# python-hydro/pyro2

Hardware: AMD Instinct MI355X
Metric: cell-updates/s (higher is better)
Workload: dtype f64; 1 GPU; compressible sedov 16384x16384 (inputs.sedov physics: HLLC, limiter 2, flattening, cvisc 0.1, cfl 0.8, outflow), one GPU, single domain (no decomposition, no halo exchange); parallelism=slab1, halo=none, fast_math=1, kernel_set=-1, dt_policy=device, state=steps 5-362 from t = 0

## Files before the change

### include/pyrohip.h

```cpp
#ifndef PYROHIP_H
#define PYROHIP_H

#include <stddef.h>

#ifdef __cplusplus
extern "C" {
#endif

typedef struct pyrohip_ctx pyrohip_ctx;
typedef struct pyrohip_state pyrohip_state;
typedef struct pyrohip_mg pyrohip_mg;

enum {
    PYROHIP_BC_OUTFLOW = 0,
    PYROHIP_BC_REFLECT_EVEN = 1,
    PYROHIP_BC_REFLECT_ODD = 2,
    PYROHIP_BC_PERIODIC = 3,
    PYROHIP_BC_HALO = 4,
    PYROHIP_BC_HSE = 5,
    PYROHIP_BC_AMBIENT = 6,
    PYROHIP_BC_RAMP = 7,
    PYROHIP_BC_CONST = 8
};

// ... 99 lines not shown
                         const double *dts, int nsteps);
int pyrohip_advrk_stage_dump(pyrohip_state *s, int var, const pyrohip_advrk_params *p, int method,
                             double dt, int stage, double *host);

typedef struct {
    double dx, dy;
    double gamma;
    int limiter;
    int use_flattening;
    double z0, z1, delta;
    double cvisc;
    double grav;
    double small_dens;
    int avisc_xhi_interior, avisc_yhi_interior;
    int fast_math;
    int kernel_set;
    int riemann, solid_xl, solid_yl;
    int do_sponge;
    double sponge_rho_begin, sponge_rho_full, sponge_timescale;
    double heat_rate;
    int march_rows;
    int fuse_fill;
    int step_launches;
} pyrohip_comp_params;

int pyrohip_comp_dt(pyrohip_state *s, const pyrohip_comp_params *p, double cfl,
                    double *dt_out);
int pyrohip_comp_step(pyrohip_state *s, const pyrohip_comp_params *p,
                      double dt);
int pyrohip_comp_wave_geometry(int nx, int ny, int ng, int num_cus, int march_rows, int *out6);
typedef struct {
    double tmax, init_tstep_factor, max_dt_change, fix_dt;
    double t, dt_old;
    long long n;
} pyrohip_dt_policy;
int pyrohip_comp_evolve(pyrohip_state *s, const pyrohip_comp_params *p, double cfl,
                        pyrohip_dt_policy *policy, int max_steps, int *steps_done,
                        double *dts_out);
int pyrohip_comp_stage_dump(pyrohip_state *s, int stage_id, double *out);

int pyrohip_mg_create(pyrohip_ctx *ctx, int nx, double xmin, double xmax,
                      double ymin, double ymax, const int *bc, double alpha,
                      double beta, int nsmooth, int nsmooth_bottom,
                      pyrohip_mg **out);
int pyrohip_mg_destroy(pyrohip_mg *m);
int pyrohip_mg_set_helmholtz(pyrohip_mg *m, double alpha, double beta);
int pyrohip_mg_nlevels(pyrohip_mg *m, int *nlevels);
int pyrohip_mg_set_smoother(pyrohip_mg *m, int kind);
typedef struct {
    int kmax, kmax_small, nsmall;
    int march_min, march_waves;
    double march_side;
    int march_minrows;
// ... 147 lines not shown
```

### pyro2_amd/_lib.py

```python
import ctypes as C
import os
import threading

import numpy as np

HERE = os.path.dirname(os.path.abspath(__file__))
DEFAULT_LIB = os.path.join(HERE, "lib", "libpyrohip.so")

BC_OUTFLOW, BC_REFLECT_EVEN, BC_REFLECT_ODD, BC_PERIODIC, BC_HALO, BC_HSE, BC_AMBIENT, BC_RAMP, \
    BC_CONST = range(9)
BC_CODE = {"outflow": BC_OUTFLOW, "neumann": BC_OUTFLOW,
           "reflect-even": BC_REFLECT_EVEN, "reflect-odd": BC_REFLECT_ODD,
           "dirichlet": BC_REFLECT_ODD, "periodic": BC_PERIODIC,
           "halo": BC_HALO, "hse": BC_HSE, "ambient": BC_AMBIENT, "ramp": BC_RAMP,
           "moving_lid": BC_CONST}

class GeomArrays(C.Structure):
    NAMES = ("Lx", "Ly", "Ax", "Ay", "V", "dlogAx", "dlogAy", "x2d", "sint", "sinb", "sinc")
    _fields_ = [(n, C.POINTER(C.c_double)) for n in NAMES] + \
               [("xmin", C.c_double), ("ymin", C.c_double),
                ("rowf", C.POINTER(C.c_double)), ("colf", C.POINTER(C.c_double))]


ERR_STATE = 10002
# ... 27 lines not shown
class MGTuning(C.Structure):
    _fields_ = [("kmax", C.c_int), ("kmax_small", C.c_int), ("nsmall", C.c_int),
                ("march_min", C.c_int), ("march_waves", C.c_int), ("march_side", C.c_double),
                ("march_minrows", C.c_int), ("fuse_res_restrict", C.c_int),
                ("lazy_residual", C.c_int), ("allow_pow2", C.c_int), ("small_tiles", C.c_int),
                ("band_maxn", C.c_int), ("band_genedge", C.c_int), ("coarse_band64", C.c_int),
                ("speculate", C.c_int), ("trace", C.c_int), ("spec_debug", C.c_int),
                ("march_tail", C.c_int), ("coarse_wave", C.c_int)]


class CompParams(C.Structure):
    _fields_ = [("dx", C.c_double), ("dy", C.c_double), ("gamma", C.c_double),
                ("limiter", C.c_int), ("use_flattening", C.c_int),
                ("z0", C.c_double), ("z1", C.c_double), ("delta", C.c_double),
                ("cvisc", C.c_double), ("grav", C.c_double),
                ("small_dens", C.c_double),
                ("avisc_xhi_interior", C.c_int),
                ("avisc_yhi_interior", C.c_int),
                ("fast_math", C.c_int), ("kernel_set", C.c_int),
                ("riemann", C.c_int), ("solid_xl", C.c_int), ("solid_yl", C.c_int),
                ("do_sponge", C.c_int), ("sponge_rho_begin", C.c_double),
                ("sponge_rho_full", C.c_double), ("sponge_timescale", C.c_double),
                ("heat_rate", C.c_double), ("march_rows", C.c_int), ("fuse_fill", C.c_int),
                ("step_launches", C.c_int)]


class DtPolicyC(C.Structure):
    _fields_ = [("tmax", C.c_double), ("init_tstep_factor", C.c_double),
                ("max_dt_change", C.c_double), ("fix_dt", C.c_double),
                ("t", C.c_double), ("dt_old", C.c_double), ("n", C.c_longlong)]


_DP = C.POINTER(C.c_double)
_IP = C.POINTER(C.c_int)
_VP = C.c_void_p

_PROTOS = {
    "pyrohip_init": [C.c_int, C.POINTER(_VP)],
    "pyrohip_shutdown": [_VP],
    "pyrohip_sync": [_VP],
    "pyrohip_device_info": [_VP, C.c_char_p, C.c_int, C.POINTER(C.c_size_t),
                            C.POINTER(C.c_size_t), _IP],
    "pyrohip_prof_enable": [_VP, C.c_int],
    "pyrohip_prof_report": [_VP, C.c_char_p, C.c_int],
    "pyrohip_timer_start": [_VP],
    "pyrohip_timer_stop": [_VP, _DP],
    "pyrohip_state_create": [_VP, C.c_int, C.c_int, C.c_int, C.c_int, _IP,
# ... 50 lines not shown
                                C.c_double, C.c_double, C.c_double, C.c_int],
    "pyrohip_inc_stage_dump": [_VP, C.c_int, _DP],
    "pyrohip_lm_set_base": [_VP, _DP, _DP, _DP, _DP],
    "pyrohip_lm_dt": [_VP, C.c_double, C.c_double, C.c_double, C.c_double, _DP],
    "pyrohip_lm_mg_coeffs": [_VP, _VP],
    "pyrohip_lm_mac_rhs": [_VP, _VP, C.c_double, C.c_double, C.c_double, C.c_int, C.c_double, _DP],
    "pyrohip_lm_advect": [_VP, _VP, C.c_double, C.c_double, C.c_double, C.c_int, C.c_int,
                          C.c_double, C.c_double],
    "pyrohip_lm_proj_rhs": [_VP, _VP, C.c_double, C.c_double, C.c_double, C.c_int, C.c_int, _DP],
    "pyrohip_lm_proj_update": [_VP, _VP, C.c_double, C.c_double, C.c_double, C.c_int],
    "pyrohip_lm_stage_dump": [_VP, C.c_int, _DP],
    "pyrohip_fill_bc": [_VP, C.c_int],
    "pyrohip_state_set_user_bc": [_VP, C.c_double, C.c_double, C.c_double, _DP],
    "pyrohip_state_set_heating": [_VP, _DP],
    "pyrohip_state_set_source": [_VP, C.c_int, _VP],
    "pyrohip_comp_source_correct": [_VP, C.POINTER(CompParams), C.c_double],
    "pyrohip_state_set_ramp_bc": [_VP, _DP, C.c_double, _DP, _DP, _DP, _DP],
    "pyrohip_state_minmax": [_VP, C.c_int, C.c_int, _DP, _DP],
    "pyrohip_adv_step": [_VP, C.c_int, C.c_double, C.c_double, C.c_double,
                         C.c_double, C.c_double, C.c_int],
    "pyrohip_adv_step_fill": [_VP, C.c_int, C.c_double, C.c_double, C.c_double,
                              C.c_double, C.c_double, C.c_int, C.c_int],
    "pyrohip_adv_step_p": [_VP, C.c_int, C.POINTER(AdvParams), C.c_double],
    "pyrohip_comp_wave_geometry": [C.c_int, C.c_int, C.c_int, C.c_int, C.c_int, C.POINTER(C.c_int)],
    "pyrohip_adv_evolve": [_VP, C.c_int, C.POINTER(AdvParams), C.POINTER(C.c_double), C.c_int],
    "pyrohip_advnu_step": [_VP, C.c_int, C.c_int, C.c_int, C.POINTER(AdvNuParams), C.c_double],
    "pyrohip_advnu_evolve": [_VP, C.c_int, C.c_int, C.c_int, C.POINTER(AdvNuParams),
                             C.POINTER(C.c_double), C.c_int],
    "pyrohip_advnu_dt": [_VP, C.c_int, C.c_int, C.c_double, C.c_double, C.c_double, _DP],
    "pyrohip_advnu_stage_dump": [_VP, C.c_int, C.c_int, C.c_int, C.POINTER(AdvNuParams), C.c_double, _DP],
    "pyrohip_advrk_rhs": [_VP, C.c_int, C.POINTER(AdvRkParams), _VP, C.c_int],
    "pyrohip_advrk_step": [_VP, C.c_int, C.POINTER(AdvRkParams), C.c_int, C.c_double],
    "pyrohip_advrk_evolve": [_VP, C.c_int, C.POINTER(AdvRkParams), C.c_int, C.POINTER(C.c_double), C.c_int],
    "pyrohip_advrk_stage_dump": [_VP, C.c_int, C.POINTER(AdvRkParams), C.c_int, C.c_double, C.c_int, _DP],
    "pyrohip_comp_dt": [_VP, C.POINTER(CompParams), C.c_double, _DP],
    "pyrohip_comp_evolve": [_VP, C.POINTER(CompParams), C.c_double, C.POINTER(DtPolicyC), C.c_int,
                            _IP, _DP],
    "pyrohip_comp_step": [_VP, C.POINTER(CompParams), C.c_double],
    "pyrohip_comp_stage_dump": [_VP, C.c_int, _DP],
    "pyrohip_mg_create": [_VP, C.c_int, C.c_double, C.c_double, C.c_double,
                          C.c_double, _IP, C.c_double, C.c_double, C.c_int,
                          C.c_int, C.POINTER(_VP)],
    "pyrohip_mg_destroy": [_VP],
    "pyrohip_mg_nlevels": [_VP, _IP],
    "pyrohip_mg_set_smoother": [_VP, C.c_int],
    "pyrohip_mg_set": [_VP, C.c_int, C.c_int, _DP],
# ... 110 lines not shown
```

### pyro2_amd/csrc/common.h

```cpp
#pragma once
#include <hip/hip_runtime.h>

#include <cstdio>
#include <cstring>
#include <string>
#include <vector>

#include "../../include/pyrohip.h"

namespace pyro {

void set_error(const std::string &msg);

#define PYRO_CHECK_HIP(expr)                                                  \
    do {                                                                      \
        hipError_t _e = (expr);                                               \
        if (_e != hipSuccess) {                                               \
            ::pyro::set_error(std::string(#expr) + ": " +                     \
                              hipGetErrorString(_e));                         \
            return (int)_e;                                                   \
        }                                                                     \
    } while (0)

#define PYRO_REQUIRE(cond, msg)                                               \
// ... 186 lines not shown
    double *heat_base = nullptr, *heat = nullptr;
    const double *ext_old = nullptr, *ext_new = nullptr;
    int ext_pending = 0;
    bool ramp_bc = false, ramp_set = false;
    double *d_x = nullptr;
    double r_cxoff = 0.0, r_post[4] = {0, 0, 0, 0}, r_pre[4] = {0, 0, 0, 0};
    double r_sfd[8] = {0}, r_sfu[8] = {0};
    double *work = nullptr;
    size_t work_planes = 0;
    int *d_flag = nullptr;
    pyro::StepScalars *d_scal = nullptr;
    double *d_dts = nullptr;
    int dts_cap = 0;
    double *pend_part = nullptr;
    int pend_n = 0;
    double *d_cval = nullptr;
    pyro::SphGeom *sph = nullptr;
    int nb_lo = -1, nb_hi = -1;
    bool nb_set = false, halo_pending = false;
    bool frame_prefilled = false;
    pyro::StepPolicy *pol_next = nullptr;
    int pol_m = 0;
    unsigned long long *d_polmem = nullptr;
    double next_cfl_min = -1.0;
    bool cfl_is_global = false;
    int cfl_kind = 0;
    double cfl_par[3] = {0.0, 0.0, 0.0};
    bool ghost_by_rules = false;
    bool stages_valid = false;
};

inline int prio_board_acquire(pyrohip_ctx *c, int **board, int *tag)
{
    const size_t bytes = (size_t)2 * 65536 * sizeof(int);
    if (c->prio_board.bytes < bytes) {
        PYRO_TRY(c->prio_board.ensure(bytes));
        PYRO_CHECK_HIP(hipMemsetAsync(c->prio_board.p, 0, bytes, c->stream));
    }
    c->launch_seq = (c->launch_seq % 32767u) + 1u;
    *board = (int *)c->prio_board.p;
    *tag = (int)c->launch_seq;
    return 0;
}
inline int wave_fill_extra(int ncb, int nsb, int nx, int slots)
{
    const int nreg = ncb * nsb;
// ... 10 lines not shown
```

### pyro2_amd/csrc/comp_api.hip

```cpp
#include "common.h"
#include "stencil.h"

namespace pyro {
namespace exact {
int comp_dt(pyrohip_state *, const pyrohip_comp_params *, double, double *);
int comp_step_staged(pyrohip_state *, const pyrohip_comp_params *, double);
int comp_step_fused(pyrohip_state *, const pyrohip_comp_params *, double);
int comp_step_wave(pyrohip_state *, const pyrohip_comp_params *, double);
int comp_step_fused_ex(pyrohip_state *, const pyrohip_comp_params *, double, const StepScalars *,
                       const double **);
int comp_step_wave_ex(pyrohip_state *, const pyrohip_comp_params *, double, const StepScalars *,
                      const double **);
int comp_cfl_min_device(pyrohip_state *, const pyrohip_comp_params *, const double **);
int comp_step_sph(pyrohip_state *, const pyrohip_comp_params *, double);
int comp_step_wave_sph(pyrohip_state *, const pyrohip_comp_params *, double);
int comp_step_wave_sph_ex(pyrohip_state *, const pyrohip_comp_params *, double, const StepScalars *,
                          const double **);
int comp_step_fused_sph(pyrohip_state *, const pyrohip_comp_params *, double);
int comp_step_fused_sph_ex(pyrohip_state *, const pyrohip_comp_params *, double, const StepScalars *,
                           const double **);
int comp_cfl_min_device_sph(pyrohip_state *, const pyrohip_comp_params *, const double **);
int comp_dt_sph(pyrohip_state *, const pyrohip_comp_params *, double, double *);
int comp_stage_dump(pyrohip_state *, int, double *);
int comp_sponge(pyrohip_state *, const pyrohip_comp_params *, double);
// ... 817 lines not shown
    PYRO_REQUIRE(dst && src && k && slots_q && cq, "NULL argument");
    PYRO_REQUIRE(dst->nvar == src->nvar && dst->g.plane == src->g.plane && dst->g.plane == k->g.plane &&
                     dst->g.nx == k->g.nx && dst->g.ny == k->g.ny,
                 "geometries differ");
    PYRO_REQUIRE(dst->ctx == src->ctx && dst->ctx == k->ctx, "states live on different contexts");
    const int nslots = k->nvar / dst->nvar;
    PYRO_REQUIRE(slot_new >= 0 && slot_new < nslots && slot_old >= 0 && slot_old < nslots,
                 "slot outside the k state");
    for (int q = 0; q < 3; q++) PYRO_REQUIRE(slots_q[q] >= 0 && slots_q[q] < nslots, "slot outside the k state");
    PYRO_TRY(exact::comp_sdc_update(dst, src, k, slot_new, slot_old, slots_q, cq, dt));
    dst->next_cfl_min = -1.0;
    dst->ghost_by_rules = false;
    return 0;
}

int pyrohip_comp_stage_dump(pyrohip_state *s, int stage_id, double *out)
{
    PYRO_REQUIRE(s && out, "NULL argument");
    return exact::comp_stage_dump(s, stage_id, out);
}

}

extern "C" int pyrohip_comp_wave_geometry(int nx, int ny, int ng, int num_cus, int march_rows, int *out6)
{
    PYRO_REQUIRE(out6 && nx > 0 && ny > 0 && ng >= 0, "bad argument");
    return pyro::exact::comp_wave_geometry(nx, ny, ng, num_cus, march_rows, out6);
}
```

### pyro2_amd/csrc/comp_fused.hip

```cpp
#include "common.h"
#include "hydro.h"
#include "reduce.h"

#ifndef PYRO_FAST
#define PYRO_FAST 0
#endif
#if PYRO_FAST
#define PYRO_NS fastm
#else
#define PYRO_NS exact
#endif

namespace pyro {
namespace PYRO_NS {

constexpr int FBI = 16;
constexpr int FBJ = 32;
constexpr int FNT = FBI * FBJ;
constexpr int FTI = FBI - 2;
constexpr int FTJ = FBJ - 2;
constexpr int FQH = FBI + 6;
constexpr int FQW = FBJ + 6;
constexpr int FQN = FQH * FQW;
constexpr int FBUF0 = (4 * FQN > 8 * FNT) ? 4 * FQN : 8 * FNT;
// ... 604 lines not shown
    P.avx_hi = p->avisc_xhi_interior; P.avy_hi = p->avisc_yhi_interior;
    P.dtdx = dt / p->dx; P.dtdy = dt / p->dy;
    P.hdtV = (0.5 * dt) / (p->dx * p->dy);
    P.dtdV = dt / (p->dx * p->dy);
    P.gm1 = p->gamma - 1.0; P.rgm1 = 1.0 / (p->gamma - 1.0);
    P.rdx = 1.0 / p->dx; P.rdy = 1.0 / p->dy;
    P.grav = p->grav;
    P.refl_ylo = (s->bc[3 * 4 + 2] == PYROHIP_BC_REFLECT_ODD);
    P.refl_yhi = (s->bc[3 * 4 + 3] == PYROHIP_BC_REFLECT_ODD);
    P.amb_yhi = (s->bc[3 * 4 + 3] == PYROHIP_BC_AMBIENT);
    P.heat = s->heat; P.heat_rate = s->heat ? p->heat_rate : 0.0;
    P.have_src = (p->grav != 0.0 || s->heat != nullptr);
    P.solid_xl = p->solid_xl; P.solid_yl = p->solid_yl;
    P.ntj = P.ntiles = 0;
    P.L = P.ncb = P.nsb = P.nunits = 0;
    P.prio_duty = 0;
    P.sb_first = 0; P.sb_step = 1; P.n_extra = 0; P.n_short = 0; P.Ls = 0; P.n_tail = 0; P.units_short = 0; P.prio_board = nullptr; P.prio_tag = 0;
    P.mr = bc_map(g.ilo, g.ihi, g.ng, 0, 0, false);
    P.mc = P.mr;
    P.odd = 0;
    P.pol = nullptr; P.pol_m = 0; P.pol_pre = 0;
    P.rk_k = nullptr; P.rk_n = 0; P.rk_a[0] = P.rk_a[1] = P.rk_a[2] = 0.0;
    P.rk_final = 0; P.rk_nb = 0; P.rk_b[0] = P.rk_b[1] = P.rk_b[2] = P.rk_b[3] = 0.0; P.rk_out = nullptr;
    if (reset_flag) PYRO_CHECK_HIP(hipMemsetAsync(s->d_flag, 0, sizeof(int), c->stream));
    return 0;
}

void fused_copy_frame(pyrohip_state *s)
{
    pyrohip_ctx *c = s->ctx;
    const Geom &g = s->g;
    const int rows_per_block = 256 / (2 * g.ng);
    const int nblk = 2 * g.ng * ((g.qy + 255) / 256) + (g.nx + rows_per_block - 1) / rows_per_block;
    hipLaunchKernelGGL(k_copy_frame4, dim3(nblk), dim3(256), 0, c->stream,
                       (const double *)s->d, s->alt_base + geom_lead(g), g);
}

int fused_tail(pyrohip_state *s, double *part, int nparts, bool frame_copied, const double **dmin_out,
               bool defer)
{
    pyrohip_ctx *c = s->ctx;
    if (!frame_copied) fused_copy_frame(s);
    if (defer && !c->global_cfl && nparts <= 128 * kMinStageBlocks) {
        s->pend_part = part;
        s->pend_n = nparts;
        *dmin_out = part + nparts + kMinStageBlocks;
// ... 156 lines not shown
```

### pyro2_amd/csrc/comp_wave.hip

```cpp
#include "common.h"
#include "hydro.h"
#include "reduce.h"

#ifndef PYRO_FAST
#define PYRO_FAST 0
#endif
#if PYRO_FAST
#define PYRO_NS fastm
#else
#define PYRO_NS exact
#endif

namespace pyro {
namespace PYRO_NS {

#include "fused_common.h"


constexpr int WOUT = 56;
#if PYRO_FAST
#define LIMIT2 half_limit2
#define SLOPE_SHARED half_slope_shared
#else
#define LIMIT2 limit2
// ... 5 lines not shown
#define STAGE_FENCE() __builtin_amdgcn_sched_barrier(0)
#endif
constexpr int WAVE_PRIO_SHIFT = 1;
constexpr int WAVE_MINW = 2;

#if !defined(PYRO_EMU)
template <int CTRL> __device__ __forceinline__ double lane_dpp(double v)
{
    int lo = __double2loint(v), hi = __double2hiint(v);
    lo = __builtin_amdgcn_mov_dpp(lo, CTRL, 0xf, 0xf, true);
    hi = __builtin_amdgcn_mov_dpp(hi, CTRL, 0xf, 0xf, true);
    return __hiloint2double(hi, lo);
}
__device__ __forceinline__ double lane_m1(double v) { return lane_dpp<0x13C>(v); }
__device__ __forceinline__ double lane_p1(double v) { return lane_dpp<0x134>(v); }
__device__ __forceinline__ double lane_m2(double v) { return lane_m1(lane_m1(v)); }
__device__ __forceinline__ double lane_p2(double v) { return lane_p1(lane_p1(v)); }
#else
__device__ __forceinline__ double lane_m1(double v) { return __shfl_up(v, 1, 64); }
__device__ __forceinline__ double lane_p1(double v) { return __shfl_down(v, 1, 64); }
__device__ __forceinline__ double lane_m2(double v) { return __shfl_up(v, 2, 64); }
__device__ __forceinline__ double lane_p2(double v) { return __shfl_down(v, 2, 64); }
#endif
__device__ __forceinline__ Cons lane_m1(const Cons &U)
{
    return Cons{lane_m1(U.d), lane_m1(U.E), lane_m1(U.mx), lane_m1(U.my)};
}
__device__ __forceinline__ Cons lane_p1(const Cons &U)
{
    return Cons{lane_p1(U.d), lane_p1(U.E), lane_p1(U.mx), lane_p1(U.my)};
}

constexpr int ST_YM = 0, ST_YP = 4, ST_FXT = 8, ST_XP = 12, ST_XPC = 16, ST_FX = 20;
constexpr int ST_L2 = 24;
constexpr int ST_AX = 32, ST_AY = 33;
constexpr int ST_XPQ = 34;
constexpr int ST_SLOTS = 37;
enum { C_GAMMA, C_DX, C_DY, C_DT, C_Z0, C_Z1, C_DELTA, C_CVISC, C_SMALLD, C_DTDX, C_DTDY, C_HDTV,
       C_DTDV, C_GRAV, C_HEATR, C_GM1, C_RGM1, C_RDX, C_RDY, C_KSL, C_KSR, C_RGP1,
       C_KX, C_KY,
       C_CX, C_CY,
       C_CVDX, C_CVDY,
       C_N };
constexpr size_t WLDS_BYTES = (size_t)(ST_SLOTS * 64 + C_N) * sizeof(double);
#define UC(name) (ct[C_##name])
#if PYRO_FAST && !defined(PYRO_EMU)
// ... 24 lines not shown
    __device__ __forceinline__ double g() const { return gam; }
    __device__ __forceinline__ double sl() const { return ct[C_KSL]; }
    __device__ __forceinline__ double sr() const { return ct[C_KSR]; }
    __device__ __forceinline__ double gp1() const { return ct[C_RGP1]; }
};

struct FlatKTab {
    UniformTab ct;
    __device__ __forceinline__ double z0() const { return ct[C_Z0]; }
    __device__ __forceinline__ double z1() const { return ct[C_Z1]; }
    __device__ __forceinline__ double delta() const { return ct[C_DELTA]; }
};

__device__ __forceinline__ Cons st_get(const double *st, int s)
{
    return Cons{st[s * 64], st[(s + 1) * 64], st[(s + 2) * 64], st[(s + 3) * 64]};
}
__device__ __forceinline__ void st_put(double *st, int s, const Cons &U)
{
    st[s * 64] = U.d; st[(s + 1) * 64] = U.E; st[(s + 2) * 64] = U.mx; st[(s + 3) * 64] = U.my;
}


#if defined(PYRO_WAVE_TIMELINE) && PYRO_FAST && !defined(PYRO_EMU)
__device__ unsigned long long g_wave_timeline[4 * 65536];
#endif
template <int SOLVER, bool STD, bool MOL = false, bool ONE = false, bool RKF = false, bool SRC = true,
          int FINT = -1, bool FB = false>
__global__ __launch_bounds__(64, WAVE_MINW) void k_ctu_wave(const double *__restrict__ Uin,
                                                                 double *__restrict__ Uout, Geom g,
                                                                 FP P, int *__restrict__ flag,
                                                                 double *__restrict__ partial,
                                                                 const StepScalars *__restrict__ S)
{
    HIP_DYNAMIC_SHARED(double, lds)
    static_assert(!RKF || (MOL && !ONE), "the folded Runge-Kutta stage is a method-of-lines launch");
    constexpr bool MAPS = ONE || RKF;
    const bool rk_final = RKF && (FINT < 0 ? P.rk_final != 0 : FINT == 1);
    const int l = threadIdx.x;
    double *st = lds + l;
    const int per = (P.nunits + 7) / 8;
    int unit = ((int)blockIdx.x % 8) * per + (int)blockIdx.x / 8;
    if (P.units_short > 0) {
        const int NL = P.nunits - P.units_short, NS = P.units_short;
        const int perL = (NL + 7) / 8, perS = (NS + 7) / 8;
        const int x = (int)blockIdx.x % 8, r = (int)blockIdx.x / 8;
// ... 5 lines not shown
    const int cb = unit < nreg ? unit % P.ncb : unit - nreg;
    const int sb = unit < nreg ? P.sb_first + (unit / P.ncb) * P.sb_step : P.nsb;
    int i0 = g.ilo + sb * P.L;
    int i1 = (sb == P.nsb - 1) ? g.ihi + 1 : i0 + P.L;
    if (cb < P.n_extra) {
        i0 = g.ilo + (int)((long)sb * g.nx / (P.nsb + 1));
        i1 = g.ilo + (int)((long)(sb + 1) * g.nx / (P.nsb + 1));
    }
    if (P.n_short > 0 && sb >= P.nsb - P.n_short - P.n_tail) {
        const int nl = P.nsb - P.n_short - P.n_tail;
        if (sb < nl + P.n_short) { i0 = g.ilo + nl * P.L + (sb - nl) * P.Ls; i1 = i0 + P.Ls; }
        else { i0 = g.ilo + nl * P.L + P.n_short * P.Ls + (sb - nl - P.n_short) * P.L; i1 = i0 + P.L; }
        if (sb == P.nsb - 1) i1 = g.ihi + 1;
    }
    const int j = g.jlo + cb * WOUT - 4 + l;
    const int jc = (j < g.qy) ? j : g.qy - 1;
    const bool jin = (j >= g.jlo && j <= g.jhi);
    const bool jout = jin && l >= 4 && l <= 59;
    const int p = g.pitch;
    const size_t pl = g.plane;
    const int limiter = STD ? 2 : P.limiter;
    const bool flat = STD || P.use_flattening;
    const bool HAVE_SRC = SRC && P.have_src;
    constexpr bool TQ = (PYRO_FAST != 0) && (SOLVER == 0) && !MOL;
    UniformTab ct = (UniformTab)(lds + ST_SLOTS * 64);
    double v_dt = P.dt, v_dtdx = P.dtdx, v_dtdy = P.dtdy, v_hdtV = P.hdtV, v_dtdV = P.dtdV;
    bool active = true;
    if (ONE) {
        StepPolicy *const pol = P.pol;
        const int m = P.pol_m;
        if (P.pol_pre) {
            const StepScalars *Sm = &pol->S[m & 1];
            v_dt = Sm->dt; v_dtdx = Sm->dtdx; v_dtdy = Sm->dtdy; v_hdtV = Sm->hdtV; v_dtdV = Sm->dtdV;
            active = Sm->active != 0;
        } else {
            StepScalars L = pol->S[(m - 1) & 1];
            const unsigned long long *prev = pol->slots + (size_t)((m - 1) % 3) * kPolSetWords;
            const double cmin = __shfl(wave_reduce_min(__longlong_as_double(
                                           (long long)prev[(size_t)l * kPolStride])), 0, 64);
            double dtm;
            dt_policy_apply(&L, cmin, (*(volatile int *)flag & (2 << ((m - 1) & 1))) != 0, &dtm, 0, 0);
            if (unit == 0) {
                atomicExch(&pol->slots[(size_t)((m + 1) % 3) * kPolSetWords + (size_t)l * kPolStride],
                           (unsigned long long)__double_as_longlong((double)INFINITY));
                if (l == 0) { pol->S[m & 1] = L; pol->dts[m] = dtm; }
            }
// ... 6 lines not shown
    }
#if defined(PYRO_WAVE_TIMELINE) && PYRO_FAST && !defined(PYRO_EMU)
    const unsigned long long tl_t0 = __builtin_amdgcn_s_memrealtime();
#endif
    auto finish = [&](double cfl, bool bad) {
        if (bad) atomicOr(flag, ONE ? (2 << (P.pol_m & 1)) : 1);
        if (l != 0) return;
#if defined(PYRO_WAVE_TIMELINE) && PYRO_FAST && !defined(PYRO_EMU)
        if (unit < 65536) {
            unsigned hwid, xcc;
            asm volatile("s_getreg_b32 %0, hwreg(HW_REG_HW_ID)" : "=s"(hwid));
            asm volatile("s_getreg_b32 %0, hwreg(HW_REG_XCC_ID)" : "=s"(xcc));
            g_wave_timeline[4 * unit] = tl_t0;
            g_wave_timeline[4 * unit + 1] = __builtin_amdgcn_s_memrealtime();
            g_wave_timeline[4 * unit + 2] = ((unsigned long long)xcc << 32) | hwid;
            g_wave_timeline[4 * unit + 3] = ((unsigned long long)sb << 32) | (unsigned)cb;
        }
#endif
        if (ONE)
            atomicMin(P.pol->slots + (size_t)(P.pol_m % 3) * kPolSetWords + (size_t)(unit % kPolSlots) * kPolStride,
                      (unsigned long long)__double_as_longlong(cfl));
        else
            partial[sb * P.ncb + cb] = cfl;
    };
    if (!active) {
        if (!ONE) finish(INFINITY, false);
        return;
    }
#if PYRO_FAST && !defined(PYRO_EMU)
    auto sgpr = [](double v) {
        return __hiloint2double(__builtin_amdgcn_readfirstlane(__double2hiint(v)),
                                __builtin_amdgcn_readfirstlane(__double2loint(v)));
    };
    const double s_dtdx = ONE ? sgpr(v_dtdx) : v_dtdx, s_dtdy = ONE ? sgpr(v_dtdy) : v_dtdy;
    const double s_hdtV = ONE ? sgpr(v_hdtV) : v_hdtV, s_dtdV = ONE ? sgpr(v_dtdV) : v_dtdV;
    const double s_kx = sgpr(-s_hdtV * P.dy), s_ky = sgpr(-s_hdtV * P.dx);
    const double s_cx = sgpr(s_dtdV * P.dy), s_cy = sgpr(s_dtdV * P.dx);
    const double s_cvdx = sgpr(P.cvisc * P.dx), s_cvdy = sgpr(P.cvisc * P.dy);
#endif
    if (l == 0) {
        ct[C_GAMMA] = P.gamma; ct[C_DX] = P.dx; ct[C_DY] = P.dy; ct[C_DT] = v_dt;
        ct[C_Z0] = P.z0; ct[C_Z1] = P.z1; ct[C_DELTA] = P.delta; ct[C_CVISC] = P.cvisc;
        ct[C_SMALLD] = P.small_dens;
        ct[C_DTDX] = v_dtdx; ct[C_DTDY] = v_dtdy;
        ct[C_HDTV] = v_hdtV; ct[C_DTDV] = v_dtdV;
        ct[C_GRAV] = P.grav; ct[C_HEATR] = P.heat_rate;
// ... 115 lines not shown

#if !defined(PYRO_EMU)
    unsigned hw_id;
    asm volatile("s_getreg_b32 %0, hwreg(HW_REG_HW_ID)" : "=s"(hw_id));
    const int wslot = (int)(hw_id & 1u);
    const bool prio_fb = FB && !MOL && P.prio_board != nullptr;
    int *prio_mine = nullptr, *prio_other = nullptr;
    int prio_seen = 0;
    if (prio_fb) {
        unsigned xcc;
        asm volatile("s_getreg_b32 %0, hwreg(HW_REG_XCC_ID)" : "=s"(xcc));
        int *const pair = P.prio_board + 2 * (int)(((xcc & 15u) << 12) | ((hw_id >> 4) & 0xfffu));
        prio_mine = pair + wslot;
        prio_other = pair + (wslot ^ 1);
    }
    auto prio_publish = [&](int k) {
        if (!prio_fb) return;
        __hip_atomic_store(prio_mine, (P.prio_tag << 16) | (i1 + 3 - k), __ATOMIC_RELAXED, __HIP_MEMORY_SCOPE_WORKGROUP);
        prio_seen = __hip_atomic_load(prio_other, __ATOMIC_RELAXED, __HIP_MEMORY_SCOPE_WORKGROUP);
    };
#else
    auto prio_publish = [](int) {};
#endif
    for (int k = i0 - 4; k <= i1 + 3; k++) {
#if !defined(PYRO_EMU)
        if (prio_fb) {
            const int seen = __builtin_amdgcn_readfirstlane(prio_seen);
            const int left = i1 + 3 - k;
            const int other_left = ((seen >> 16) == P.prio_tag) ? (seen & 0xffff) : left;
            if (left > other_left) __builtin_amdgcn_s_setprio(1);
            else if (left < other_left) __builtin_amdgcn_s_setprio(0);
        } else
        if (P.prio_duty > 0) {
            const int phase = ((k - i0) >> WAVE_PRIO_SHIFT) & 7;
            if (wslot ? (phase < P.prio_duty) : (phase >= P.prio_duty)) __builtin_amdgcn_s_setprio(1);
            else __builtin_amdgcn_s_setprio(0);
        }
#endif
#pragma unroll
        for (int n = 0; n < 4; n++) {
            wr[n] = wr[n + 1]; wu[n] = wu[n + 1]; wv[n] = wv[n + 1]; wp[n] = wp[n + 1];
        }
        if (DELAY)
            Uem = prim_to_cons_g(Prim{wr[0], wu[0], wv[0], wp[0]}, US(GM1, P.gm1), US(RGM1, P.rgm1));
        else
        Uem = Ue;
        if (NOREP) {
            Ue = prim_to_cons_g(Prim{wr[1], wu[1], wv[1], wp[1]}, US(GM1, P.gm1), US(RGM1, P.rgm1));
        } else {
        Ue = Urep;
        addK(Ue, Krep);
        fix_sign(Ue, k - 3);
        if (row_in(k - 3) && jin) Ue.d = fmax(Ue.d, US(SMALLD, P.small_dens));
        }
        if (!NOREP) { Urep = loadU(k - 2); Krep = loadK(k - 2); }
        {
            Cons U = Upre;
            addK(U, Kpre);
            fix_sign(U, k);
            if (!DELAY) {
            Upre = loadU(k + 1);
// ... 314 lines not shown
                        cfl_speeds(Y, US(GAMMA, P.gamma), ax, ay);
                        st[ST_AX * 64] = fmax(st[ST_AX * 64], pdiv(ax, dxx) + pdiv(ay, dyy));
                    } else {
                    Uout[kr] = Un.d; Uout[pl + kr] = Un.E; Uout[2 * pl + kr] = Un.mx;
                    Uout[3 * pl + kr] = Un.my;
                    }
                } else {
#if PYRO_FAST
                const double cx = US(CX, s_cx), cy = US(CY, s_cy);
                Un.d = fma(cx, Fxp.d - Fxn.d, fma(cy, Fy.d - Fyh.d, Uc.d));
                Un.E = fma(cx, Fxp.E - Fxn.E, fma(cy, Fy.E - Fyh.E, Uc.E));
                Un.mx = fma(cx, Fxp.mx - Fxn.mx, fma(cy, Fy.mx - Fyh.mx, Uc.mx));
                Un.my = fma(cx, Fxp.my - Fxn.my, fma(cy, Fy.my - Fyh.my, Uc.my));
#else
                const double dtdV = UC(DTDV), Ax = UC(DY);
                Un.d = Uc.d + dtdV * (Fxp.d * Ax - Fxn.d * Ax + Fy.d * Ay - Fyh.d * Ay);
                Un.E = Uc.E + dtdV * (Fxp.E * Ax - Fxn.E * Ax + Fy.E * Ay - Fyh.E * Ay);
                Un.mx = Uc.mx + dtdV * (Fxp.mx * Ax - Fxn.mx * Ax + Fy.mx * Ay - Fyh.mx * Ay);
                Un.my = Uc.my + dtdV * (Fxp.my * Ax - Fxn.my * Ax + Fy.my * Ay - Fyh.my * Ay);
#endif
                const size_t ko = (size_t)(i - 1) * p + j;
                if (HAVE_SRC)
                    grav_update(Un, Uc, UC(GRAV), UC(DT), UC(HEATR), P.heat ? P.heat[ko] : 0.0);
                if (DELAY) {
                    Upend = Un;
                } else if (SADDR) {
                    const unsigned off = (unsigned)(i - 1 - rbase) * pitch8 + (unsigned)j * 8u;
                    *(double *)(sbase_out + off) = Un.d; *(double *)(sbase_out + plb + off) = Un.E;
                    *(double *)(sbase_out + 2 * plb + off) = Un.mx; *(double *)(sbase_out + 3 * plb + off) = Un.my;
                } else {
                Uout[ko] = Un.d; Uout[pl + ko] = Un.E; Uout[2 * pl + ko] = Un.mx;
                Uout[3 * pl + ko] = Un.my;
                }
                double ax, ay;
                cfl_speeds(Un, US(GAMMA, P.gamma), ax, ay);
                st[ST_AX * 64] = fmax(st[ST_AX * 64], ax);
                st[ST_AY * 64] = fmax(st[ST_AY * 64], ay);
                }
            }
            if (xface) st_put(st, ST_FX, Fxn);
        }
        fxa = fxb; fxb = fxn;
        Dp = Dn; up = um; vp = vm;
    }
    if (DELAY && i1 + 3 >= i0 + 4 && jout) {
        const unsigned off = (unsigned)(i1 - 1 - rbase) * pitch8 + (unsigned)j * 8u;
        *(double *)(sbase_out + off) = Upend.d; *(double *)(sbase_out + plb + off) = Upend.E;
        *(double *)(sbase_out + 2 * plb + off) = Upend.mx; *(double *)(sbase_out + 3 * plb + off) = Upend.my;
    }
    if (bad) atomicOr(flag, 1);
    const double ax = st[ST_AX * 64], ay = st[ST_AY * 64];
    double cfl = fmin(ax > 0.0 ? pdiv(P.dx, ax) : INFINITY, ay > 0.0 ? pdiv(P.dy, ay) : INFINITY);
    if (RKF) cfl = ax > 0.0 ? pdiv(1.0, ax) : INFINITY;
    finish(__shfl(wave_reduce_min(cfl), 0, 64), bad);
}

static int wave_rows(int nx, int ncb, int slots)
{
    if (nx <= 32) return nx;
    long best_cost = -1;
    int best = 32;
    for (int L = 8; L <= 160 && L <= nx; L++) {
        int nsb = (nx + L - 1) / L;
        if (nsb > 1 && nx - (nsb - 1) * L < 4) nsb--;
// ... 51 lines not shown
    *Ls = ls; *nsb_long = nl;
    return ns;
}
#if !PYRO_FAST
int comp_wave_geometry(int nx, int ny, int ng, int cus, int march_rows, int *out)
{
    const WaveGeom w = wave_geometry(nx, ny, ng, cus > 0 ? cus : 256, march_rows);
    out[0] = w.ncb; out[1] = w.L; out[2] = w.nsb; out[3] = w.overlap;
    out[4] = w.ncb * w.nsb; out[5] = 4 * WAVE_MINW * (cus > 0 ? cus : 256);
    return 0;
}
#endif

int comp_step_wave_ex(pyrohip_state *s, const pyrohip_comp_params *p, double dt,
                      const StepScalars *S, const double **dmin_out)
{
    pyrohip_ctx *c = s->ctx;
    const Geom &g = s->g;
    FP P;
    double *Uin, *Uout;
    PYRO_TRY(fused_prepare(s, p, dt, P, Uin, Uout, S == nullptr));
    const int cus = c->num_cus > 0 ? c->num_cus : 256;
    const WaveGeom wg = wave_geometry(g.nx, g.ny, g.ng, cus, p->march_rows);
    P.ncb = wg.ncb;
    P.L = wg.L;
    const int nsb = wg.nsb;
    P.nsb = nsb;
    const bool post = s->nb_set && comm_can_overlap(s);
    P.n_extra = (s->nb_set || post) ? 0 : wave_extra_units(wg, g.nx, 4 * WAVE_MINW * cus, p->march_rows);
    int nsb_long = nsb;
    if (!s->nb_set && !post && !(S && s->pol_next))
        P.n_short = wave_short_tail(wg, g.nx, 4 * WAVE_MINW * cus, p->march_rows, &P.Ls, &nsb_long);
    if (P.n_short > 0) { P.nsb = nsb_long + P.n_short; P.units_short = P.ncb * P.n_short; }
    int slab_short = 0;
    if (post && wg.overlap) {
        int ls = 0, nl1 = 0;
        const int ns1 = wave_short_tail(wg, g.nx, 4 * WAVE_MINW * cus, 0, &ls, &nl1);
        const int div = ls > 0 ? (P.L + ls - 1) / ls : 0;
        const int nr = nsb - nl1;
        if (ns1 > 0 && div >= 2 && P.L % div == 0 && nsb - nr - 1 >= 2) {
            P.Ls = P.L / div;
            P.n_short = nr * div;
            P.n_tail = 1;
            P.nsb = nsb + nr * (div - 1);
            slab_short = P.ncb * P.n_short;
        }
// ... 243 lines not shown
```

### pyro2_amd/csrc/ctx.hip

```cpp
#include "common.h"
#include "reduce.h"

namespace pyro {

static thread_local std::string g_last_error;
void set_error(const std::string &msg) { g_last_error = msg; }

int DevBuf::ensure(size_t need)
{
    if (need <= bytes) return 0;
    if (p) PYRO_CHECK_HIP(hipFree(p));
    p = nullptr; bytes = 0;
    PYRO_CHECK_HIP(hipMalloc(&p, need));
    bytes = need;
    return 0;
}
void DevBuf::release()
{
    if (p) (void)hipFree(p);
    p = nullptr; bytes = 0;
}

__global__ void k_aos_to_planar(const double *__restrict__ aos, double *__restrict__ d,
                                int i0, int ni, int qy, int nvar, int pitch, size_t plane)
// ... 395 lines not shown
    s->bc.assign(bc, bc + nvar * 4);
    size_t n = s->g.plane * nvar + 16;
    PYRO_CHECK_HIP(hipMalloc((void **)&s->base, n * sizeof(double)));
    PYRO_CHECK_HIP(hipMemsetAsync(s->base, 0, n * sizeof(double), c->stream));
    s->d = s->base + geom_lead(s->g);
    PYRO_CHECK_HIP(hipMalloc((void **)&s->d_bc, sizeof(int) * nvar * 4));
    PYRO_CHECK_HIP(hipMemcpy(s->d_bc, bc, sizeof(int) * nvar * 4, hipMemcpyHostToDevice));
    PYRO_CHECK_HIP(hipMalloc((void **)&s->d_cval, sizeof(double) * nvar));
    PYRO_CHECK_HIP(hipMemsetAsync(s->d_cval, 0, sizeof(double) * nvar, c->stream));
    PYRO_CHECK_HIP(hipMalloc((void **)&s->d_flag, sizeof(int) * 4));
    PYRO_CHECK_HIP(hipMemsetAsync(s->d_flag, 0, sizeof(int) * 4, c->stream));
    *out = s;
    return 0;
}

int pyrohip_state_destroy(pyrohip_state *s)
{
    if (!s) return 0;
    (void)hipSetDevice(s->ctx->device);
    (void)comm_wait_halo(s);
    (void)hipStreamSynchronize(s->ctx->stream);
    if (s->d_scal) (void)hipFree(s->d_scal);
    if (s->d_polmem) (void)hipFree(s->d_polmem);
    if (s->d_dts) (void)hipFree(s->d_dts);
    if (s->base) (void)hipFree(s->base);
    if (s->alt_base) (void)hipFree(s->alt_base);
    if (s->d_bc) (void)hipFree(s->d_bc);
    if (s->d_x) (void)hipFree(s->d_x);
    if (s->heat_base) (void)hipFree(s->heat_base);
    if (s->d_flag) (void)hipFree(s->d_flag);
    if (s->d_cval) (void)hipFree(s->d_cval);
    if (s->sph) { if (s->sph->base) (void)hipFree(s->sph->base); delete s->sph; }
    if (s->work) (void)hipFree(s->work);
    delete s;
    return 0;
}

static const size_t kStageBytes = (size_t)256 << 20;

static int rows_per_chunk(const pyrohip_state *s)
{
    size_t row = (size_t)s->g.qy * s->nvar * sizeof(double);
    size_t r = kStageBytes / row;
    if (r < 1) r = 1;
    return (int)r;
}
// ... 376 lines not shown
```

### pyro2_amd/csrc/fused_common.h

```cpp
#pragma once

struct FP {
    double gamma, dx, dy, dt;
    double z0, z1, delta, cvisc, small_dens;
    int limiter, use_flattening;
    int avx_hi, avy_hi;
    int ntj, ntiles;
    double dtdx, dtdy;
    double hdtV;
    double dtdV;
    double gm1, rgm1;
    double rdx, rdy;
    double grav;
    int refl_ylo, refl_yhi;
    int amb_yhi;
    int have_src;
    double heat_rate;
    const double *heat;
    int solid_xl, solid_yl;
    int L, ncb, nsb;
    int nunits;
    int prio_duty;
    int sb_first, sb_step;
    int n_extra;
    int n_short, Ls;
    int n_tail, units_short;
    int *prio_board;
    int prio_tag;
    BcMap mr, mc;
    unsigned odd;
    StepPolicy *pol;
    int pol_m;
    int pol_pre;
    const double *rk_k;
    int rk_n;
    double rk_a[3];
    int rk_final;
    int rk_nb;
    double rk_b[4];
    double *rk_out;
};

__device__ __forceinline__ bool odd_sides(unsigned m)
{
    m &= 15u;
    m ^= m >> 2;
    m ^= m >> 1;
    return (m & 1u) != 0;
}

__global__ void k_copy_frame4(const double *__restrict__ src, double *__restrict__ dst, Geom g);
int fused_prepare(pyrohip_state *s, const pyrohip_comp_params *p, double dt, FP &P, double *&Uin,
                  double *&Uout, bool reset_flag = true, bool second_buffer = true);
int fused_tail(pyrohip_state *s, double *part, int nparts, bool frame_copied, const double **dmin,
               bool defer = false);
int fused_sync(pyrohip_state *s, const double *dmin);
void fused_swap(pyrohip_state *s);
void fused_copy_frame(pyrohip_state *s);

__device__ __forceinline__ ConsN to_nf(const Cons &U, bool x)
{
    return x ? ConsN{U.d, U.E, U.mx, U.my} : ConsN{U.d, U.E, U.my, U.mx};
}
// ... 96 lines not shown
```

### pyro2_amd/device.py

```python
import ctypes as C
import threading

import numpy as np

from . import _lib
from ._lib import BC_CODE, CompParams, check, dptr, iptr


def comp_wave_geometry(nx, ny, ng=4, num_cus=0, march_rows=0):
    out = (C.c_int * 6)()
    check(_lib.lib().pyrohip_comp_wave_geometry(int(nx), int(ny), int(ng), int(num_cus),
                                                  int(march_rows), out))
    return dict(zip(("col_strips", "rows_per_strip", "row_strips", "overlap", "wavefronts", "slots"),
                    (int(v) for v in out)))


def _check_run(rc, dts):
    try:
        check(rc)
    except _lib.PyroHipError as e:
        e.steps_done, e.dts = len(dts), dts
        raise


# ... 522 lines not shown
            check(self._l.pyrohip_comp_dt(self.h, C.byref(params), cfl, C.byref(dt)))
        return dt.value

    def comp_dt_is_cached(self):
        f = C.c_int()
        check(self._l.pyrohip_comp_dt_is_cached(self.h, C.byref(f)))
        return bool(f.value)

    def comp_rk_dt_is_cached(self):
        f = C.c_int()
        with self.ctx.lock:
            check(self._l.pyrohip_comp_rk_dt_is_cached(self.h, C.byref(f)))
        return bool(f.value)

    def comp_dt_is_global(self):
        f = C.c_int()
        check(self._l.pyrohip_comp_dt_is_global(self.h, C.byref(f)))
        return bool(f.value)

    def comp_step(self, params, dt):
        with self.ctx.lock:
            check(self._l.pyrohip_comp_step(self.h, C.byref(params), dt))

    def set_source(self, which, src):
        with self.ctx.lock:
            check(self._l.pyrohip_state_set_source(self.h, int(which), src.h if src is not None else None))
        self._src = getattr(self, "_src", {})
        self._src[which] = src

    def comp_source_correct(self, params, dt):
        with self.ctx.lock:
            check(self._l.pyrohip_comp_source_correct(self.h, C.byref(params), dt))

    def comp_rk_can_fuse(self, params, kstate, nstages):
        f = C.c_int()
        with self.ctx.lock:
            check(self._l.pyrohip_comp_rk_can_fuse(self.h, C.byref(params), kstate.h, int(nstages), C.byref(f)))
        return bool(f.value)

    def comp_rk_step(self, params, kstate, dt, a, b):
        a = np.ascontiguousarray(a, dtype=np.float64)
        b = np.ascontiguousarray(b, dtype=np.float64)
        with self.ctx.lock:
            check(self._l.pyrohip_comp_rk_step(self.h, C.byref(params), kstate.h, float(dt), len(b),
                                               dptr(a), dptr(b)))

# ... 44 lines not shown
    def halo_pending(self):
        f = C.c_int()
        check(self._l.pyrohip_state_halo_pending(self.h, C.byref(f)))
        return bool(f.value)

    def halo_exchange(self, rank_lo, rank_hi):
        with self.ctx.lock:
            check(self._l.pyrohip_halo_exchange(self.h, int(rank_lo), int(rank_hi)))

    def send_rows(self, i0, ni, peer):
        with self.ctx.lock:
            check(self._l.pyrohip_state_send_rows(self.h, int(i0), int(ni), int(peer)))

    def recv_rows(self, i0, ni, peer):
        with self.ctx.lock:
            check(self._l.pyrohip_state_recv_rows(self.h, int(i0), int(ni), int(peer)))


def make_comp_params(dx, dy, gamma=1.4, limiter=2, use_flattening=1, z0=0.75,
                     z1=0.85, delta=0.33, cvisc=0.1, grav=0.0,
                     small_dens=-1.e200, avisc_xhi_interior=0,
                     avisc_yhi_interior=0, fast_math=0, kernel_set=0, riemann="HLLC",
                     solid_xl=0, solid_yl=0, sponge=None, heat_rate=0.0, march_rows=0,
                     fuse_fill=0, step_launches=0):
    p = CompParams()
    p.dx, p.dy, p.gamma = dx, dy, gamma
    p.limiter, p.use_flattening = int(limiter), int(use_flattening)
    p.z0, p.z1, p.delta, p.cvisc = z0, z1, delta, cvisc
    p.grav, p.small_dens = grav, small_dens
    p.avisc_xhi_interior = int(avisc_xhi_interior)
    p.avisc_yhi_interior = int(avisc_yhi_interior)
    p.fast_math, p.kernel_set = int(fast_math), int(kernel_set)
    p.riemann = {"HLLC": 0, "CGF": 1, "HLLC_lm": 2}[riemann] if isinstance(riemann, str) else int(riemann)
    p.solid_xl, p.solid_yl = int(solid_xl), int(solid_yl)
    if sponge is not None:
        p.do_sponge = 1
        p.sponge_rho_begin, p.sponge_rho_full, p.sponge_timescale = sponge
    p.heat_rate = float(heat_rate)
    p.march_rows = int(march_rows)
    p.fuse_fill = int(fuse_fill)
    p.step_launches = int(step_launches)
    return p


class DeviceMG:

    def __init__(self, ctx, nx, xmin=0.0, xmax=1.0, ymin=0.0, ymax=1.0,
                 bcs=("dirichlet",) * 4, alpha=0.0, beta=-1.0, nsmooth=10,
                 nsmooth_bottom=50, tuning=None):
        self.ctx = ctx
        self._l = ctx._l
        bc = np.array([BC_CODE[b] if isinstance(b, str) else int(b) for b in bcs],
                      dtype=np.int32)
        self.h = C.c_void_p()
        with ctx.lock:
            check(self._l.pyrohip_mg_create(ctx.h, int(nx), xmin, xmax, ymin, ymax,
                                            iptr(bc), alpha, beta, int(nsmooth),
                                            int(nsmooth_bottom), C.byref(self.h)))
            nl = C.c_int()
            check(self._l.pyrohip_mg_nlevels(self.h, C.byref(nl)))
        self.nx = int(nx)
        self.nlevels = nl.value
        self.dx = (xmax - xmin) / nx
        self.source_norm = 0.0
# ... 164 lines not shown
```

Measured before the change: 31.99 billion cell-updates/s.

## Skip wave-row updates over uniform flat regions in wave-march kernel

Adds a wavefront-uniform detection in the row-marching compressible kernel. When all 64 lanes hold bit-identical state across several consecutive rows, and the previous update was verified to be an identity, the kernel copies the input row to the output instead of running reconstruction and the Riemann solve. This targets the large quiescent ambient region in Sedov, at the cost of ballot checks each row and extra register pressure. An optional device counter records how many rows were skipped.

After: 75.54 billion cell-updates/s, median of 6. 2.36x the previous value.

```diff
diff --git a/include/pyrohip.h b/include/pyrohip.h
--- a/include/pyrohip.h
+++ b/include/pyrohip.h
@@ -145,6 +145,7 @@
     int march_rows;
     int fuse_fill;
     int step_launches;
+    int flat_skip;
 } pyrohip_comp_params;
 
 int pyrohip_comp_dt(pyrohip_state *s, const pyrohip_comp_params *p, double cfl,
@@ -152,6 +153,7 @@
 int pyrohip_comp_step(pyrohip_state *s, const pyrohip_comp_params *p,
                       double dt);
 int pyrohip_comp_wave_geometry(int nx, int ny, int ng, int num_cus, int march_rows, int *out6);
+int pyrohip_comp_wave_flat_rows(pyrohip_state *s, long long *out);
 typedef struct {
     double tmax, init_tstep_factor, max_dt_change, fix_dt;
     double t, dt_old;
diff --git a/pyro2_amd/_lib.py b/pyro2_amd/_lib.py
--- a/pyro2_amd/_lib.py
+++ b/pyro2_amd/_lib.py
@@ -73,7 +73,7 @@
                 ("do_sponge", C.c_int), ("sponge_rho_begin", C.c_double),
                 ("sponge_rho_full", C.c_double), ("sponge_timescale", C.c_double),
                 ("heat_rate", C.c_double), ("march_rows", C.c_int), ("fuse_fill", C.c_int),
-                ("step_launches", C.c_int)]
+                ("step_launches", C.c_int), ("flat_skip", C.c_int)]
 
 
 class DtPolicyC(C.Structure):
@@ -170,6 +170,7 @@
     "pyrohip_adv_step_fill": [_VP, C.c_int, C.c_double, C.c_double, C.c_double,
                               C.c_double, C.c_double, C.c_int, C.c_int],
     "pyrohip_adv_step_p": [_VP, C.c_int, C.POINTER(AdvParams), C.c_double],
+    "pyrohip_comp_wave_flat_rows": [_VP, C.POINTER(C.c_longlong)],
     "pyrohip_comp_wave_geometry": [C.c_int, C.c_int, C.c_int, C.c_int, C.c_int, C.POINTER(C.c_int)],
     "pyrohip_adv_evolve": [_VP, C.c_int, C.POINTER(AdvParams), C.POINTER(C.c_double), C.c_int],
     "pyrohip_advnu_step": [_VP, C.c_int, C.c_int, C.c_int, C.POINTER(AdvNuParams), C.c_double],
diff --git a/pyro2_amd/csrc/common.h b/pyro2_amd/csrc/common.h
--- a/pyro2_amd/csrc/common.h
+++ b/pyro2_amd/csrc/common.h
@@ -232,6 +232,7 @@
     pyro::StepPolicy *pol_next = nullptr;
     int pol_m = 0;
     unsigned long long *d_polmem = nullptr;
+    unsigned long long *flat_rows = nullptr;
     double next_cfl_min = -1.0;
     bool cfl_is_global = false;
     int cfl_kind = 0;
diff --git a/pyro2_amd/csrc/comp_api.hip b/pyro2_amd/csrc/comp_api.hip
--- a/pyro2_amd/csrc/comp_api.hip
+++ b/pyro2_amd/csrc/comp_api.hip
@@ -863,6 +863,24 @@
 
 }
 
+extern "C" int pyrohip_comp_wave_flat_rows(pyrohip_state *s, long long *out)
+{
+    PYRO_REQUIRE(s, "NULL argument");
+    pyrohip_ctx *c = s->ctx;
+    PYRO_CHECK_HIP(hipSetDevice(c->device));
+    PYRO_CHECK_HIP(hipStreamSynchronize(c->stream));
+    if (!out) {
+        if (s->flat_rows) PYRO_CHECK_HIP(hipFree(s->flat_rows));
+        s->flat_rows = nullptr;
+        return 0;
+    }
+    *out = 0;
+    if (!s->flat_rows) PYRO_CHECK_HIP(hipMalloc((void **)&s->flat_rows, sizeof(unsigned long long)));
+    else PYRO_CHECK_HIP(hipMemcpy(out, s->flat_rows, sizeof(long long), hipMemcpyDeviceToHost));
+    PYRO_CHECK_HIP(hipMemset(s->flat_rows, 0, sizeof(unsigned long long)));
+    return 0;
+}
+
 extern "C" int pyrohip_comp_wave_geometry(int nx, int ny, int ng, int num_cus, int march_rows, int *out6)
 {
     PYRO_REQUIRE(out6 && nx > 0 && ny > 0 && ng >= 0, "bad argument");
diff --git a/pyro2_amd/csrc/comp_fused.hip b/pyro2_amd/csrc/comp_fused.hip
--- a/pyro2_amd/csrc/comp_fused.hip
+++ b/pyro2_amd/csrc/comp_fused.hip
@@ -650,6 +650,7 @@
     P.pol = nullptr; P.pol_m = 0; P.pol_pre = 0;
     P.rk_k = nullptr; P.rk_n = 0; P.rk_a[0] = P.rk_a[1] = P.rk_a[2] = 0.0;
     P.rk_final = 0; P.rk_nb = 0; P.rk_b[0] = P.rk_b[1] = P.rk_b[2] = P.rk_b[3] = 0.0; P.rk_out = nullptr;
+    P.flat_skip = -1; P.flat_rows = nullptr;
     if (reset_flag) PYRO_CHECK_HIP(hipMemsetAsync(s->d_flag, 0, sizeof(int), c->stream));
     return 0;
 }
diff --git a/pyro2_amd/csrc/comp_wave.hip b/pyro2_amd/csrc/comp_wave.hip
--- a/pyro2_amd/csrc/comp_wave.hip
+++ b/pyro2_amd/csrc/comp_wave.hip
@@ -51,6 +51,28 @@
 __device__ __forceinline__ double lane_m2(double v) { return __shfl_up(v, 2, 64); }
 __device__ __forceinline__ double lane_p2(double v) { return __shfl_down(v, 2, 64); }
 #endif
+#if !defined(PYRO_EMU)
+__device__ __forceinline__ bool wave_all(bool p) { return __builtin_amdgcn_ballot_w64(p) == ~0ull; }
+__device__ __forceinline__ bool wave_none4(bool a, bool b, bool c, bool d)
+{
+    return (__builtin_amdgcn_ballot_w64(a) | __builtin_amdgcn_ballot_w64(b) | __builtin_amdgcn_ballot_w64(c) |
+            __builtin_amdgcn_ballot_w64(d)) == 0ull;
+}
+__device__ __forceinline__ long long wave_first_bits(double v)
+{
+    const unsigned lo = (unsigned)__builtin_amdgcn_readfirstlane(__double2loint(v));
+    const unsigned hi = (unsigned)__builtin_amdgcn_readfirstlane(__double2hiint(v));
+    return (long long)(((unsigned long long)hi << 32) | lo);
+}
+#else
+__device__ __forceinline__ bool wave_all(bool p) { return __shfl(wave_reduce_min(p ? 1.0 : 0.0), 0, 64) != 0.0; }
+__device__ __forceinline__ bool wave_none4(bool a, bool b, bool c, bool d) { return wave_all(!(a | b | c | d)); }
+__device__ __forceinline__ long long wave_first_bits(double v) { return __double_as_longlong(__shfl(v, 0, 64)); }
+#endif
+__device__ __forceinline__ bool same_bits(double a, double b)
+{
+    return __double_as_longlong(a) == __double_as_longlong(b);
+}
 __device__ __forceinline__ Cons lane_m1(const Cons &U)
 {
     return Cons{lane_m1(U.d), lane_m1(U.E), lane_m1(U.mx), lane_m1(U.my)};
@@ -121,6 +143,7 @@
 }
 
 
+constexpr int FLAT_DEPTH = 10;
 #if defined(PYRO_WAVE_TIMELINE) && PYRO_FAST && !defined(PYRO_EMU)
 __device__ unsigned long long g_wave_timeline[4 * 65536];
 #endif
@@ -172,6 +195,9 @@
     const int limiter = STD ? 2 : P.limiter;
     const bool flat = STD || P.use_flattening;
     const bool HAVE_SRC = SRC && P.have_src;
+    constexpr bool FLATK = !MOL && !ONE && !RKF && !(PYRO_FAST != 0 && SRC) && !(SOLVER == 2 && STD);
+    const bool flat_on = FLATK && !HAVE_SRC && P.flat_skip >= 0;
+    int fskip = 0;
     constexpr bool TQ = (PYRO_FAST != 0) && (SOLVER == 0) && !MOL;
     UniformTab ct = (UniformTab)(lds + ST_SLOTS * 64);
     double v_dt = P.dt, v_dtdx = P.dtdx, v_dtdy = P.dtdy, v_hdtV = P.hdtV, v_dtdV = P.dtdV;
@@ -224,6 +250,7 @@
                       (unsigned long long)__double_as_longlong(cfl));
         else
             partial[sb * P.ncb + cb] = cfl;
+        if (FLATK && P.flat_rows) atomicAdd(P.flat_rows, (unsigned long long)fskip);
     };
     if (!active) {
         if (!ONE) finish(INFINITY, false);
@@ -385,6 +412,13 @@
 #else
     auto prio_publish = [](int) {};
 #endif
+    long long fF[4] = {0, 0, 0, 0};
+    int fcnt = 0;
+    bool farm = false;
+    if (FLATK && flat_on) {
+        fF[0] = wave_first_bits(Upre.d); fF[1] = wave_first_bits(Upre.E);
+        fF[2] = wave_first_bits(Upre.mx); fF[3] = wave_first_bits(Upre.my);
+    }
     for (int k = i0 - 4; k <= i1 + 3; k++) {
 #if !defined(PYRO_EMU)
         if (prio_fb) {
@@ -400,6 +434,43 @@
             else __builtin_amdgcn_s_setprio(0);
         }
 #endif
+        if (FLATK && flat_on) {
+            const bool same = wave_none4(__double_as_longlong(Upre.d) != fF[0], __double_as_longlong(Upre.E) != fF[1],
+                                         __double_as_longlong(Upre.mx) != fF[2], __double_as_longlong(Upre.my) != fF[3]);
+            if (same) {
+                if (farm && k <= g.ihi) {
+                    const Cons Un{Upre.d + 0.0, Upre.E + 0.0, Upre.mx + 0.0, Upre.my + 0.0};
+                    if (DELAY) {
+                        if (jout) {
+                            const unsigned off = (unsigned)(k - 5 - rbase) * pitch8 + (unsigned)j * 8u;
+                            *(double *)(sbase_out + off) = Upend.d; *(double *)(sbase_out + plb + off) = Upend.E;
+                            *(double *)(sbase_out + 2 * plb + off) = Upend.mx; *(double *)(sbase_out + 3 * plb + off) = Upend.my;
+                        }
+                        Upend = Un;
+                    } else if (jout) {
+                        if (SADDR) {
+                            const unsigned off = (unsigned)(k - 4 - rbase) * pitch8 + (unsigned)j * 8u;
+                            *(double *)(sbase_out + off) = Un.d; *(double *)(sbase_out + plb + off) = Un.E;
+                            *(double *)(sbase_out + 2 * plb + off) = Un.mx; *(double *)(sbase_out + 3 * plb + off) = Un.my;
+                        } else {
+                            const size_t ko = (size_t)(k - 4) * p + j;
+                            Uout[ko] = Un.d; Uout[pl + ko] = Un.E; Uout[2 * pl + ko] = Un.mx; Uout[3 * pl + ko] = Un.my;
+                        }
+                    }
+                    Upre = loadU(k + 1);
+                    prio_publish(k);
+                    fskip++;
+                    continue;
+                }
+                fcnt++;
+            } else {
+                fF[0] = wave_first_bits(Upre.d); fF[1] = wave_first_bits(Upre.E);
+                fF[2] = wave_first_bits(Upre.mx); fF[3] = wave_first_bits(Upre.my);
+                fcnt = 0;
+                farm = false;
+            }
+        }
+        bool fid = true;
 #pragma unroll
         for (int n = 0; n < 4; n++) {
             wr[n] = wr[n + 1]; wu[n] = wu[n + 1]; wv[n] = wv[n + 1]; wp[n] = wp[n + 1];
@@ -760,6 +831,9 @@
                 const size_t ko = (size_t)(i - 1) * p + j;
                 if (HAVE_SRC)
                     grav_update(Un, Uc, UC(GRAV), UC(DT), UC(HEATR), P.heat ? P.heat[ko] : 0.0);
+                if (FLATK && flat_on && fcnt >= FLAT_DEPTH - 1)
+                    fid = same_bits(Un.d, Uc.d + 0.0) && same_bits(Un.E, Uc.E + 0.0) &&
+                          same_bits(Un.mx, Uc.mx + 0.0) && same_bits(Un.my, Uc.my + 0.0);
                 if (DELAY) {
                     Upend = Un;
                 } else if (SADDR) {
@@ -778,6 +852,13 @@
             }
             if (xface) st_put(st, ST_FX, Fxn);
         }
+        if (FLATK && flat_on) {
+            farm = false;
+            if (fcnt >= FLAT_DEPTH - 1 && k >= i0 + 5) {
+                const double Fd = __longlong_as_double(fF[0]);
+                farm = positive_finite_bits(Fd) && Fd >= P.small_dens && wave_all(fid);
+            }
+        }
         fxa = fxb; fxb = fxn;
         Dp = Dn; up = um; vp = vm;
     }
@@ -875,6 +956,8 @@
     PYRO_TRY(fused_prepare(s, p, dt, P, Uin, Uout, S == nullptr));
     const int cus = c->num_cus > 0 ? c->num_cus : 256;
     const WaveGeom wg = wave_geometry(g.nx, g.ny, g.ng, cus, p->march_rows);
+    P.flat_skip = p->flat_skip < 0 ? -1 : 0;
+    P.flat_rows = s->flat_rows;
     P.ncb = wg.ncb;
     P.L = wg.L;
     const int nsb = wg.nsb;
diff --git a/pyro2_amd/csrc/ctx.hip b/pyro2_amd/csrc/ctx.hip
--- a/pyro2_amd/csrc/ctx.hip
+++ b/pyro2_amd/csrc/ctx.hip
@@ -441,6 +441,7 @@
     (void)hipStreamSynchronize(s->ctx->stream);
     if (s->d_scal) (void)hipFree(s->d_scal);
     if (s->d_polmem) (void)hipFree(s->d_polmem);
+    if (s->flat_rows) (void)hipFree(s->flat_rows);
     if (s->d_dts) (void)hipFree(s->d_dts);
     if (s->base) (void)hipFree(s->base);
     if (s->alt_base) (void)hipFree(s->alt_base);
diff --git a/pyro2_amd/csrc/fused_common.h b/pyro2_amd/csrc/fused_common.h
--- a/pyro2_amd/csrc/fused_common.h
+++ b/pyro2_amd/csrc/fused_common.h
@@ -39,6 +39,8 @@
     int rk_nb;
     double rk_b[4];
     double *rk_out;
+    int flat_skip;
+    unsigned long long *flat_rows;
 };
 
 __device__ __forceinline__ bool odd_sides(unsigned m)
diff --git a/pyro2_amd/device.py b/pyro2_amd/device.py
--- a/pyro2_amd/device.py
+++ b/pyro2_amd/device.py
@@ -568,6 +568,12 @@
         with self.ctx.lock:
             check(self._l.pyrohip_comp_step(self.h, C.byref(params), dt))
 
+    def comp_wave_flat_rows(self, disarm=False):
+        n = C.c_longlong(0)
+        with self.ctx.lock:
+            check(self._l.pyrohip_comp_wave_flat_rows(self.h, None if disarm else C.byref(n)))
+        return n.value
+
     def set_source(self, which, src):
         with self.ctx.lock:
             check(self._l.pyrohip_state_set_source(self.h, int(which), src.h if src is not None else None))
@@ -658,7 +664,7 @@
                      small_dens=-1.e200, avisc_xhi_interior=0,
                      avisc_yhi_interior=0, fast_math=0, kernel_set=0, riemann="HLLC",
                      solid_xl=0, solid_yl=0, sponge=None, heat_rate=0.0, march_rows=0,
-                     fuse_fill=0, step_launches=0):
+                     fuse_fill=0, step_launches=0, flat_skip=0):
     p = CompParams()
     p.dx, p.dy, p.gamma = dx, dy, gamma
     p.limiter, p.use_flattening = int(limiter), int(use_flattening)
@@ -676,6 +682,7 @@
     p.march_rows = int(march_rows)
     p.fuse_fill = int(fuse_fill)
     p.step_launches = int(step_launches)
+    p.flat_skip = int(flat_skip)
     return p
 
 
```
